# bransonf/mosaic

Hardware: AMD Instinct MI355X
Metric: PIP-join points/sec (whole node) at H3 res 9, 1/2/4/8 MI355X vs CPU host (higher is better)
Workload: dtype f64

## Files before the change

mosaic_amd/csrc/join_binned.h:

```cpp
#pragma once
#include <hip/hip_runtime.h>
#include <stddef.h>
#include <stdint.h>

#include <vector>

#include "join_common.h"
#include "tile_images.h"

namespace binned {

struct Pt {
    double x, y;
};
struct PtRow {
    double x, y;
    long long row;
};
__host__ __device__ inline void set_row(Pt&, int64_t) {}
__host__ __device__ inline void set_row(PtRow& p, int64_t r) { p.row = (long long)r; }
__host__ __device__ inline int64_t row_of(const Pt&, int64_t i) { return i; }
__host__ __device__ inline int64_t row_of(const PtRow& p, int64_t) { return (int64_t)p.row; }
inline const long long* row_map(const Pt*) { return nullptr; }
inline const long long* row_map(const PtRow* p) { return &p->row; }
// ... 47 lines not shown

#define MOSAIC_FP_MIX(h, v) ((h) * 0x100000001b3ULL ^ (uint64_t)(v))
static constexpr uint64_t mosaic_layout_fingerprint() {
    uint64_t h = 0xcbf29ce484222325ULL;
    h = MOSAIC_FP_MIX(h, sizeof(JoinArgs));
    h = MOSAIC_FP_MIX(h, sizeof(StreamArgs));
    h = MOSAIC_FP_MIX(h, sizeof(BngStreamArgs));
    h = MOSAIC_FP_MIX(h, sizeof(binned::Scratch));
    h = MOSAIC_FP_MIX(h, offsetof(binned::Scratch, exact_args));
    h = MOSAIC_FP_MIX(h, offsetof(binned::Scratch, sorted_rows));
    h = MOSAIC_FP_MIX(h, offsetof(binned::Scratch, spin_cap));
    h = MOSAIC_FP_MIX(h, offsetof(binned::Scratch, lookback_failed));
    h = MOSAIC_FP_MIX(h, sizeof(binned::Images));
    h = MOSAIC_FP_MIX(h, offsetof(JoinArgs, res));
    h = MOSAIC_FP_MIX(h, offsetof(JoinArgs, counts));
    return h;
}
#undef MOSAIC_FP_MIX
```

mosaic_amd/csrc/join_common.h:

```cpp
#pragma once
#include <hip/hip_runtime.h>
#include <stdint.h>

#include "bng_device.h"
#include "pip_device.h"
#include "raster.h"
#include "tiles.h"

using namespace mosaic;

static const int64_t kEmptyKey = INT64_MIN;

struct HashEntry {
    int64_t key;
    uint32_t first;
    uint32_t count;
};

__host__ __device__ inline uint64_t mix64(uint64_t h) {
    h ^= h >> 33;
    h *= 0xff51afd7ed558ccdULL;
    h ^= h >> 33;
    h *= 0xc4ceb9fe1a85ec53ULL;
    h ^= h >> 33;
// ... 99 lines not shown
        atomicAdd(&a.counts[key], 1ULL);
    if (PAIRS) {
        unsigned long long idx = atomicAdd(a.pair_count, 1ULL);
        if ((long long)idx < a.pair_cap) {
            a.pair_row[idx] = row;
            a.pair_key[idx] = (int)key;
        }
    }
}

__device__ inline void stage_push(uint32_t* wq, uint32_t& wn, bool mixed, uint32_t rowoff, unsigned long long lt_mask) {
    const unsigned long long mm = __ballot(mixed);
    if (mixed) wq[wn + __popcll(mm & lt_mask)] = rowoff;
    wn += (uint32_t)__popcll(mm);
}
__device__ inline void stage_flush(const JoinArgs& a, uint32_t* wq, uint32_t& wn, int lane, uint32_t min_rows) {
    if (wn < min_rows || wn == 0) return;
    __builtin_amdgcn_fence(__ATOMIC_RELEASE, "wavefront");
    __builtin_amdgcn_wave_barrier();
    __builtin_amdgcn_fence(__ATOMIC_ACQUIRE, "wavefront");
    unsigned long long base = 0;
    if (lane == 0) base = atomicAdd(a.mixq_count, (unsigned long long)wn);
    base = __shfl(base, 0, 64);
    for (uint32_t k = (uint32_t)lane; k < wn; k += 64) a.mixq[base + k] = wq[k];
    __builtin_amdgcn_wave_barrier();
    wn = 0;
}

struct StreamArgs {
    double x0, y0, sxC, syC;
    double gxmax, gymax;
    int32_t cs, qsh, tsh, qs;
    int32_t qnx, tnx;
    int32_t n_quad_words, n_tiles;
    int32_t tb_lds;
    int32_t stage_words;
    const uint32_t* quad;
    const uint32_t* tile_base;
    const uint16_t* csub;
    const uint16_t* blocks;
    uint32_t csub_bytes, blocks_bytes, tile_base_bytes;
    const uint32_t* qrec;
    int32_t n_qrec, n_qrec_words, qrl;
    double sxF, syF, gx0F, gy0F;
    int32_t gxmaxF, gymaxF, fix_ok;
    const uint32_t* tile_lbase;
    const tiles::LineRec* llines;
};
static const int kStageWords = 128;
static const int kCptBufWords = 192;
static const uint32_t kNoLoad = 0x7ffffff0u;

typedef double v2d __attribute__((ext_vector_type(2)));
typedef unsigned int v4u __attribute__((ext_vector_type(4)));

__device__ inline void lds_fill(uint32_t* dst, const uint32_t* __restrict__ src, int n) {
    const int nt = (int)blockDim.x;
    int k = (int)threadIdx.x;
    for (; k + 7 * nt < n; k += 8 * nt) {
        uint32_t v[8];
#pragma unroll
        for (int j = 0; j < 8; j++) v[j] = src[k + j * nt];
#pragma unroll
        for (int j = 0; j < 8; j++) dst[k + j * nt] = v[j];
// ... 14 lines not shown
    return r;
}

template <int SH0 = 0>
__device__ inline uint32_t quad_lookup(const StreamArgs& s, const uint16_t* quad, const uint32_t* qmask,
                                       const uint16_t* qcode, uint32_t ixC, uint32_t iyC) {
    const uint32_t q = quad[mad_u24(iyC >> (s.qsh + SH0), (uint32_t)s.qnx, ixC >> (s.qsh + SH0))];
    const uint32_t r = q - 0x8000u;
    const bool rec = r < (uint32_t)s.n_qrec;
    const uint32_t sh = (uint32_t)(s.cs + s.qrl + SH0);
    const uint32_t b = (__builtin_amdgcn_ubfe(iyC, sh, 3u) << 3) | __builtin_amdgcn_ubfe(ixC, sh, 3u);
    const uint32_t rr = rec ? r : 0u;
    const uint32_t w = qmask[2u * rr + (b >> 5)];
    const uint32_t c = qcode[rr];
    return (rec && __builtin_amdgcn_ubfe(w, b & 31u, 1u)) ? c : q;
}

static const uint32_t kBngPure = 0x80000000u, kBngLeaf = 0x40000000u;
static const uint32_t kBngLdsGather = 0xFFu;
struct BngStreamArgs {
    int32_t e0, n0, ne, nn, C;
    double inv_div, div, f;
    int32_t idiv;
    float ff;
    const uint32_t* cells;
    const uint16_t* leaf;
    uint32_t cells_bytes, leaf_bytes;
    const uint32_t* lcell;
    int32_t lcell_words, lsh, lnx;
    const uint16_t* lvl;
// ... 8 lines not shown
```

mosaic_amd/csrc/join_stream.hip:

```cpp
#include "join_binned.h"
#include "join_common.h"

template <bool LDS_COUNTS, bool PAIRS, bool VEC>
__global__ void __launch_bounds__(1024) __attribute__((amdgpu_waves_per_eu(4))) k_join_stream(JoinArgs a, StreamArgs s) {
    extern __shared__ unsigned int lds[];
    const int nwaves = (int)(blockDim.x >> 6);
    const int ncw = LDS_COUNTS ? a.n_polygons + 64 : 0;
    uint32_t* stage = lds + ncw;
    uint32_t* tb = stage + nwaves * s.stage_words;
    uint32_t* quadw = tb + (s.tb_lds ? s.n_tiles : 0);
    const uint16_t* quad = (const uint16_t*)quadw;
    uint32_t* qmask = quadw + s.n_quad_words;
    const uint16_t* qcode = (const uint16_t*)(qmask + 2 * s.n_qrec);
    lds_fill(quadw, s.quad, s.n_quad_words);
    lds_fill(qmask, s.qrec, s.n_qrec_words);
    if (s.tb_lds)
        lds_fill(tb, s.tile_base, s.n_tiles);
    for (int k = threadIdx.x; k < ncw; k += blockDim.x) lds[k] = 0;
    __syncthreads();
    const __amdgpu_buffer_rsrc_t rsub = stream_rsrc(s.csub, s.csub_bytes);
    const __amdgpu_buffer_rsrc_t rblk = stream_rsrc(s.blocks, s.blocks_bytes);
    const __amdgpu_buffer_rsrc_t rtb = stream_rsrc(s.tile_base, s.tile_base_bytes);
    const int lane = (int)(threadIdx.x & 63);
    const unsigned long long lt_mask = (1ULL << lane) - 1ULL;
    const int wave = __builtin_amdgcn_readfirstlane((int)(threadIdx.x >> 6));
    uint32_t* wq = stage + wave * s.stage_words;
    uint32_t wn = 0;
    const uint32_t cm = (1u << s.cs) - 1u, qm = (1u << s.qs) - 1u, tm = (1u << s.tsh) - 1u;
    const int64_t stride = (int64_t)gridDim.x * blockDim.x * 4;
    int64_t w0 = a.row_lo + ((int64_t)blockIdx.x * blockDim.x + (int64_t)wave * 64) * 4;
    auto row_of = [&](int64_t wb, int k) -> int64_t { return wb + (k >> 1) * 128 + 2 * lane + (k & 1); };
    v2d px[2], py[2];
    auto load4 = [&](int64_t wb) {
        const int64_t r = (wb + 256 <= a.n) ? wb + 2 * lane : a.row_lo;
        px[0] = __builtin_nontemporal_load((const v2d*)(a.x + r));
        px[1] = __builtin_nontemporal_load((const v2d*)(a.x + r + 128));
        py[0] = __builtin_nontemporal_load((const v2d*)(a.y + r));
        py[1] = __builtin_nontemporal_load((const v2d*)(a.y + r + 128));
    };
    if (VEC) load4(w0);
    for (; w0 < a.n; w0 += stride) {
        const bool full = VEC && w0 + 256 <= a.n;
// ... 68 lines not shown
#pragma unroll
        for (int k = 0; k < 4; k++) {
            if (LDS_COUNTS && !PAIRS) {
                const uint32_t slot = code[k] - 1u < 0xfffeu ? code[k] - 1u : (uint32_t)(a.n_polygons + lane);
                atomicAdd(&lds[slot], 1u);
            } else if (code[k] - 1u < 0xfffeu) {
                emit_hit<LDS_COUNTS, PAIRS>(a, row_of(w0, k), code[k] - 1u, lds);
            }
        }
        const bool anym = code[0] == tiles::kMixed || code[1] == tiles::kMixed || code[2] == tiles::kMixed ||
                          code[3] == tiles::kMixed;
        if (__ballot(anym)) {
#pragma unroll
            for (int k = 0; k < 4; k++) {
                const bool m = code[k] == tiles::kMixed;
                const unsigned long long mm = __ballot(m);
                if (m) wq[wn + __popcll(mm & lt_mask)] = (uint32_t)(row_of(w0, k) - a.row_lo);
                wn += (uint32_t)__popcll(mm);
                stage_flush(a, wq, wn, lane, 64);
            }
        }
    }
    stage_flush(a, wq, wn, lane, 1);
    if (LDS_COUNTS) {
        __syncthreads();
        for (int k = threadIdx.x; k < a.n_polygons; k += blockDim.x)
            if (lds[k]) atomicAdd(&a.counts[k], (unsigned long long)lds[k]);
    }
}


template <int aux>
__device__ inline uint32_t gather_b16(__amdgpu_buffer_rsrc_t r, bool need, uint32_t off) {
    uint32_t v = 0u;
    if (need) v = __builtin_amdgcn_raw_buffer_load_b16(r, off, 0, aux);
    return v;
}
__device__ inline uint32_t gather_b32(__amdgpu_buffer_rsrc_t r, bool need, uint32_t off) {
// ... 12 lines not shown
    uint32_t gx[4], gy[4];
    uint32_t tbv[4];
    uint32_t qv[4];
    uint32_t code[4];
    uint32_t leaf[4];
    v4u lrec[4];
};
static const uint32_t kPipeNonFinite = 0x7fffu;
static_assert(tiles::kMaxRasterKeys + 1 < 0x7fff, "key codes stay below kPipeNonFinite");
static const uint32_t kPipeLine = 0x10000u;

template <bool LDS_COUNTS, bool PAIRS>
__global__ void __launch_bounds__(1024) __attribute__((amdgpu_waves_per_eu(4))) k_join_stream_pipe(JoinArgs a, StreamArgs s) {
    extern __shared__ unsigned int lds[];
    const int nwaves = (int)(blockDim.x >> 6);
    const int ncw = LDS_COUNTS ? a.n_polygons + 64 : 0;
    uint32_t* stage = lds + ncw;
    uint32_t* tb = stage + nwaves * s.stage_words;
    uint32_t* quadw = tb + s.n_tiles;
    const uint16_t* quad = (const uint16_t*)quadw;
    uint32_t* qmask = quadw + s.n_quad_words;
    const uint16_t* qcode = (const uint16_t*)(qmask + 2 * s.n_qrec);
    lds_fill(quadw, s.quad, s.n_quad_words);
    lds_fill(qmask, s.qrec, s.n_qrec_words);
    lds_fill(tb, s.tile_base, s.n_tiles);
    for (int k = threadIdx.x; k < ncw; k += blockDim.x) lds[k] = 0;
    __syncthreads();
    const __amdgpu_buffer_rsrc_t rsub = stream_rsrc(s.csub, s.csub_bytes);
    const __amdgpu_buffer_rsrc_t rblk = stream_rsrc(s.blocks, s.blocks_bytes);
    const int lane = (int)(threadIdx.x & 63);
    const unsigned long long lt_mask = (1ULL << lane) - 1ULL;
    const int wave = __builtin_amdgcn_readfirstlane((int)(threadIdx.x >> 6));
    uint32_t* wq = stage + wave * s.stage_words;
    uint32_t wn = 0;
    const uint32_t cm = (1u << s.cs) - 1u, qm = (1u << s.qs) - 1u;
    const double gx0 = -s.x0 * s.sxC, gy0 = -s.y0 * s.syC;
    const uint32_t spill = (uint32_t)(a.n_polygons + lane);
    const int64_t stride = (int64_t)gridDim.x * blockDim.x * 4;
    const int64_t wbase = a.row_lo + ((int64_t)blockIdx.x * blockDim.x + (int64_t)wave * 64) * 4;
    const int64_t T = wbase + 256 <= a.n ? (a.n - 256 - wbase) / stride + 1 : 0;
    auto row_of = [&](int64_t wb, int k) -> int64_t { return wb + (k >> 1) * 128 + 2 * lane + (k & 1); };
    auto stage_a = [&](const double* x, const double* y, const bool* live, bool valid, PipeGroup& g) {
#pragma unroll
        for (int k = 0; k < 4; k++) {
            const bool lv = valid && live[k];
            const uint32_t ixC = min(tiles::fix_cvt(fma(x[k], s.sxF, s.gx0F)), (uint32_t)s.gxmaxF);
            const uint32_t iyC = min(tiles::fix_cvt(fma(y[k], s.syF, s.gy0F)), (uint32_t)s.gymaxF);
            g.gx[k] = ixC;
            g.gy[k] = iyC;
// ... 39 lines not shown
        }
#pragma unroll
        for (int k = 0; k < 4; k++) {
            if (LDS_COUNTS && !PAIRS) {
                const uint32_t slot = min(code[k] - 1u, spill);
                atomicAdd(&lds[slot], 1u);
            } else if (code[k] - 1u < kPipeNonFinite - 1u) {
                emit_hit<LDS_COUNTS, PAIRS>(a, row_of(wb, k), code[k] - 1u, lds);
            }
        }
        const uint32_t cmax = max(max(code[0], code[1]), max(code[2], code[3]));
        if (__ballot(cmax >= kPipeNonFinite)) {
#pragma unroll
            for (int k = 0; k < 4; k++) {
                const bool m = code[k] >= kPipeNonFinite;
                const unsigned long long mm = __ballot(m);
                if (m) wq[wn + __popcll(mm & lt_mask)] = (uint32_t)(row_of(wb, k) - a.row_lo);
                wn += (uint32_t)__popcll(mm);
                stage_flush(a, wq, wn, lane, 64);
            }
        }
    };
    struct Coords {
        v2d px[2], py[2];
    };
    auto load4 = [&](Coords& cb, int64_t wb, bool valid) {
        const int64_t r = valid ? wb + 2 * lane : wbase + 2 * lane;
        cb.px[0] = __builtin_nontemporal_load((const v2d*)(a.x + r));
        cb.px[1] = __builtin_nontemporal_load((const v2d*)(a.x + r + 128));
        cb.py[0] = __builtin_nontemporal_load((const v2d*)(a.y + r));
        cb.py[1] = __builtin_nontemporal_load((const v2d*)(a.y + r + 128));
    };
    Coords cb0, cb1;
    PipeGroup g0, g1;
// ... 35 lines not shown
    if (wt < a.n) {
        double x[4], y[4];
        bool live[4];
#pragma unroll
        for (int k = 0; k < 4; k++) {
            const int64_t r = row_of(wt, k);
            live[k] = r < a.n;
            x[k] = live[k] ? a.x[r] : 0.0;
            y[k] = live[k] ? a.y[r] : 0.0;
        }
        PipeGroup g;
        stage_a(x, y, live, true, g);
        stage_b(g);
        stage_d(g, wt);
    }
    stage_flush(a, wq, wn, lane, 1);
    if (LDS_COUNTS) {
        __syncthreads();
        for (int k = threadIdx.x; k < a.n_polygons; k += blockDim.x)
            if (lds[k]) atomicAdd(&a.counts[k], (unsigned long long)lds[k]);
    }
}


struct CptSet {
    uint32_t a;
    uint32_t b;
    uint32_t c;
    uint32_t code;
    uint32_t leaf;
    v4u lrec;
};

template <bool LDS_COUNTS, bool PAIRS>
__global__ void __launch_bounds__(1024) __attribute__((amdgpu_waves_per_eu(4))) k_join_stream_cpt(JoinArgs a, StreamArgs s) {
    extern __shared__ unsigned int lds[];
    const int nwaves = (int)(blockDim.x >> 6);
    const int ncw = LDS_COUNTS ? a.n_polygons + 64 : 0;
    uint32_t* stage = lds + ncw;
    uint32_t* cbuf_all = stage + nwaves * s.stage_words;
    uint32_t* tb = cbuf_all + nwaves * kCptBufWords;
    uint32_t* quadw = tb + (s.tb_lds ? s.n_tiles : 0);
    const uint16_t* quad = (const uint16_t*)quadw;
    uint32_t* qmask = quadw + s.n_quad_words;
    const uint16_t* qcode = (const uint16_t*)(qmask + 2 * s.n_qrec);
    lds_fill(quadw, s.quad, s.n_quad_words);
    lds_fill(qmask, s.qrec, s.n_qrec_words);
    if (s.tb_lds) lds_fill(tb, s.tile_base, s.n_tiles);
    for (int k = threadIdx.x; k < ncw; k += blockDim.x) lds[k] = 0;
    __syncthreads();
    const __amdgpu_buffer_rsrc_t rsub = stream_rsrc(s.csub, s.csub_bytes);
    const __amdgpu_buffer_rsrc_t rblk = stream_rsrc(s.blocks, s.blocks_bytes);
    const __amdgpu_buffer_rsrc_t rtb = stream_rsrc(s.tile_base, s.tile_base_bytes);
// ... 60 lines not shown
        if (MOSAIC_ABL_GATHER_HIT & 9) z.lrec = v4u{0u, 0u, __float_as_uint(2.0f), 0x00010001u};
        if (MOSAIC_ABL_GATHER_HIT & 10) z.leaf = z.code == kPipeLine ? z.leaf : 1u;
#endif
        const float u = (float)__builtin_amdgcn_ubfe(z.a, 0u, fb) * (1.0f / (float)(1 << F));
        const float v = (float)__builtin_amdgcn_ubfe(z.b, 0u, fb) * (1.0f / (float)(1 << F));
        const float sv = fmaf(__uint_as_float(z.lrec.x), u, fmaf(__uint_as_float(z.lrec.y), v, __uint_as_float(z.lrec.z)));
        const uint32_t pos = z.lrec.w & 0xffffu, neg = z.lrec.w >> 16;
        uint32_t lc = sv >= 1.0f ? pos : (uint32_t)tiles::kMixed;
        lc = sv <= -1.0f ? neg : lc;
        const uint32_t code = z.code == kPipeLine ? lc : (z.code | z.leaf);
        const uint32_t src = (z.a >> 24) & 63u, k = z.a >> 30;
        const int64_t row = wb + (int64_t)((k >> 1) * 128u + 2u * src + (k & 1u));
        answer(code, row);
        const bool m = code >= kPipeNonFinite;
        if (__ballot(m)) {
            const unsigned long long mm = __ballot(m);
            if (m) wq[wn + __popcll(mm & lt_mask)] = (uint32_t)(row - a.row_lo);
            wn += (uint32_t)__popcll(mm);
            stage_flush(a, wq, wn, lane, 64);
        }
    };
    auto stage_a = [&](const double* x, const double* y, const bool* live, bool valid, CptSet& z, CptSet& z2, bool& two,
                       int64_t wb) {
        uint32_t fa[4], fb[4], fc[4];
        bool pend[4];
#pragma unroll
        for (int k = 0; k < 4; k++) {
            const uint32_t ixC = min(tiles::fix_cvt(fma(x[k], s.sxF, gx0v)), (uint32_t)s.gxmaxF);
            const uint32_t iyC = min(tiles::fix_cvt(fma(y[k], s.syF, gy0v)), (uint32_t)s.gymaxF);
            const uint32_t q0 = quad_lookup<F>(s, quad, qmask, qcode, ixC, iyC);
            const uint32_t q = valid && live[k] ? q0 : 0u;
            const uint32_t tile = mad_u24(iyC >> (s.tsh + F), (uint32_t)s.tnx, ixC >> (s.tsh + F));
            if (LDS_COUNTS && !PAIRS) atomicAdd(&lds[min(q - 1u, spill)], 1u);
            else if (q - 1u < kPipeNonFinite - 1u) emit_hit<LDS_COUNTS, PAIRS>(a, wb + (k >> 1) * 128 + 2 * lane + (k & 1), q - 1u, lds);
// ... 102 lines not shown
            const int64_t r = wt + (k >> 1) * 128 + 2 * lane + (k & 1);
            live[k] = r < a.n;
            x[k] = live[k] ? a.x[r] : 0.0;
            y[k] = live[k] ? a.y[r] : 0.0;
        }
        CptSet z, z2;
        bool two = false;
        stage_a(x, y, live, true, z, z2, two, wt);
        set_b(z);
        set_d(z, wt);
        if (two) {
            set_b(z2);
            set_d(z2, wt);
        }
    }
    stage_flush(a, wq, wn, lane, 1);
    if (LDS_COUNTS) {
        __syncthreads();
        for (int k = threadIdx.x; k < a.n_polygons; k += blockDim.x)
            if (lds[k]) atomicAdd(&a.counts[k], (unsigned long long)lds[k]);
    }
}

template <bool LDS_COUNTS, bool PAIRS, bool VEC>
__global__ void __launch_bounds__(1024) __attribute__((amdgpu_waves_per_eu(4))) k_join_stream_bng(JoinArgs a, BngStreamArgs s) {
    extern __shared__ unsigned int lds[];
    const int ncw = LDS_COUNTS ? a.n_polygons + 64 : 0;
    uint32_t* stage = lds + ncw;
    uint32_t* lcw = stage + (int)(blockDim.x >> 6) * kStageWords;
    const uint8_t* lcell = (const uint8_t*)lcw;
    const bool use_lc = s.lcell_words > 0;
// ... 368 lines not shown
        for (int k = threadIdx.x; k < a.n_polygons; k += blockDim.x)
            if (lds[k]) atomicAdd(&a.counts[k], (unsigned long long)lds[k]);
    }
}

template <bool LDS_COUNTS, bool PAIRS>
__global__ void __launch_bounds__(256) k_join_leaf(JoinArgs a, StreamArgs s, uint32_t* q2, unsigned long long* q2_count) {
    extern __shared__ unsigned int lds[];
    if (LDS_COUNTS) {
        for (int k = threadIdx.x; k < a.n_polygons; k += blockDim.x) lds[k] = 0;
        __syncthreads();
    }
    JoinArgs aq = a;
    aq.mixq = q2;
    aq.mixq_count = q2_count;
    uint32_t* wq = lds + (LDS_COUNTS ? a.n_polygons : 0) + (threadIdx.x >> 6) * kStageWords;
    uint32_t wn = 0;
    constexpr int F = tiles::kFixBits;
    const int lane = (int)(threadIdx.x & 63);
    const unsigned long long lt_mask = (1ULL << lane) - 1ULL;
    const uint16_t* quad = (const uint16_t*)s.quad;
    const uint32_t* qmask = s.qrec;
    const uint16_t* qcode = (const uint16_t*)(s.qrec + 2 * s.n_qrec);
    const uint32_t cs = (uint32_t)s.cs, qs = (uint32_t)s.qs, cm = (1u << cs) - 1u, qm = (1u << qs) - 1u;
    const unsigned long long total = *a.mixq_count;
    const unsigned long long stride = (unsigned long long)gridDim.x * blockDim.x;
    for (unsigned long long t0 = (unsigned long long)blockIdx.x * blockDim.x + (threadIdx.x & ~63u); t0 < total; t0 += stride) {
        const unsigned long long t = t0 + (unsigned long long)lane;
        const bool live = t < total;
        const uint32_t off = live ? a.mixq[t] : 0u;
        const int64_t row = a.row_lo + (int64_t)off;
        uint32_t code = tiles::kMixed;
        if (live) {
            const double x = a.x[row], y = a.y[row];
            if (isfinite(x + y)) {
                const uint32_t gix = min(tiles::fix_cvt(fma(x, s.sxF, s.gx0F)), (uint32_t)s.gxmaxF);
                const uint32_t giy = min(tiles::fix_cvt(fma(y, s.syF, s.gy0F)), (uint32_t)s.gymaxF);
                const uint32_t ixC = gix >> F, iyC = giy >> F, ix = ixC >> cs, iy = iyC >> cs;
                const uint32_t q = quad_lookup<F>(s, quad, qmask, qcode, gix, giy);
                const uint32_t e = q < 0x8000u ? q : s.csub[((q & 0x7fffu) << (2 * qs)) + (((iy & qm) << qs) | (ix & qm))];
                code = e;
                if (tiles::sub_is_block(e) && !(e & tiles::kLineBit)) {
                    const uint32_t tile = (iyC >> s.tsh) * (uint32_t)s.tnx + (ixC >> s.tsh);
                    const uint32_t base = s.tile_base[tile];
                    const uint32_t lc = s.blocks[base + ((e & 0x3fffu) << (2 * cs)) + (((iyC & cm) << cs) | (ixC & cm))];
                    code = lc;
                    if (tiles::leaf_is_line(lc)) {
                        const tiles::LineRec lr = s.llines[s.tile_lbase[tile] + (lc & 0x3fffu)];
                        const uint32_t fm = (1u << (cs + F)) - 1u;
                        const float sc = 1.0f / (float)(1 << F);
                        code = tiles::line_code(lr, (float)(gix & fm) * sc, (float)(giy & fm) * sc);
                    }
                } else if (tiles::sub_is_block(e)) {
                    code = tiles::kMixed;
                }
            }
        }
        const bool keep = live && code >= 0x8000u;
        if (live && !keep && code != 0u) {
            if (LDS_COUNTS && !PAIRS) atomicAdd(&lds[code - 1u], 1u);
            else emit_hit<LDS_COUNTS, PAIRS>(a, row, code - 1u, lds);
        }
        stage_push(wq, wn, keep, off, lt_mask);
        stage_flush(aq, wq, wn, lane, 64);
    }
    stage_flush(aq, wq, wn, lane, 1);
    if (LDS_COUNTS) {
        __syncthreads();
        for (int k = threadIdx.x; k < a.n_polygons; k += blockDim.x)
            if (lds[k]) atomicAdd(&a.counts[k], (unsigned long long)lds[k]);
    }
}

const void* leaf_kernel(bool lds, bool pairs) {
    if (pairs) return (const void*)k_join_leaf<false, true>;
    if (lds) return (const void*)k_join_leaf<true, false>;
    return (const void*)k_join_leaf<false, false>;
}

// ... 29 lines not shown
```

mosaic_amd/csrc/mosaic_hip.hip:

```cpp
#include <hip/hip_runtime.h>
#include <hipcub/hipcub.hpp>
#include <stdint.h>
#include <stdio.h>
#include <string.h>

#include <sys/syscall.h>
#include <unistd.h>

#include <algorithm>
#include <atomic>
#include <chrono>
#include <memory>
#include <mutex>
#include <numeric>
#include <string>
#include <sys/mman.h>
#include <dirent.h>
#include <sys/prctl.h>
#include <thread>
#include <unordered_map>
#include <vector>

#include "../../include/mosaic_hip.h"
#include "bng_device.h"
// ... 1785 lines not shown
    int block = 256;
    int blocks_per_cu = 8;
    int raster = 16;
    int raster_adaptive = 1;
    int raster_min_segments = 0;
    int lane_edges = 0;
    int tiles = 1;
    int point_raster = 1;
    int raster_sub = 64;
    int raster_cell = 16;
    int raster_quad = 1;
    int raster_lines = 1;
    int raster_tb_lds = 1;
    int raster_leaf_lines = 1;
    int leaf_join = 1;
    int leaf_blocks_per_cu = 2;
    int exact_defer = 0;
    int raster_build = 1;
    int raster_quad_records = 1;
    int stream_block = 1024;
    int bng_cpt = 1;
    int stream_pipe = 2;
    int bng_lds = 1;
    int bng_cell = 32;
    int bng_group_lines = 1;
    int bng_wedges = 1;
    int cell_blocks_per_cu = 256;
    int mixed_blocks_per_cu = 16;
    int mixed_rows = 1;
    int64_t host_chunk = (int64_t)1 << 25;
    int timing = 0;
// ... 538 lines not shown
        o.raster_quad = (int)v;
    } else if (k == "raster_adaptive") {
        o.raster_adaptive = v ? 1 : 0;
    } else if (k == "raster_min_segments") {
        if (v < 0 || v > 1000000) return fail(MOSAIC_E_ARG, "raster_min_segments must be in [0, 1e6]");
        o.raster_min_segments = (int)v;
    } else if (k == "raster_lines") {
        o.raster_lines = v ? 1 : 0;
    } else if (k == "raster_tb_lds") {
        if (v < 0 || v > 2) return fail(MOSAIC_E_ARG, "raster_tb_lds must be 0, 1 or 2");
        o.raster_tb_lds = (int)v;
    } else if (k == "raster_leaf_lines") {
        o.raster_leaf_lines = v ? 1 : 0;
    } else if (k == "leaf_join") {
        o.leaf_join = v ? 1 : 0;
    } else if (k == "exact_defer") {
        o.exact_defer = v ? 1 : 0;
    } else if (k == "leaf_blocks_per_cu") {
        if (v < 1 || v > 64) return fail(MOSAIC_E_ARG, "leaf_blocks_per_cu must be in [1, 64]");
        o.leaf_blocks_per_cu = (int)v;
    } else if (k == "raster_quad_records") {
        o.raster_quad_records = v ? 1 : 0;
    } else if (k == "raster_build") {
        if (v < 0 || v > 2) return fail(MOSAIC_E_ARG, "raster_build must be 0 (host), 1 (GPU) or 2 (GPU, lane-per-sub-block lines)");
        o.raster_build = (int)v;
    } else if (k == "host_chunk") {
        if (v < 0) return fail(MOSAIC_E_ARG, "host_chunk must be >= 0");
        o.host_chunk = v;
    } else if (k == "stream_block") {
        if (v < 64 || v > 1024 || v % 64) return fail(MOSAIC_E_ARG, "stream_block must be a multiple of 64 in [64, 1024]");
// ... 1644 lines not shown
    a.rowmap = nullptr;
    bool lds = ch->n_polygons <= kLdsCountsMax;
    size_t shm = lds ? (size_t)ch->n_polygons * 4 : 0;
    int g = grid_size(c, n);
    bool binned_used = false, exact_inline = false;
    if (n > 0) {
        hipEvent_t tstop;
        if ((rc = timing_begin(c, &tstop))) return rc;
        const bool h3g = ch->grid == MOSAIC_GRID_H3;
#define MOSAIC_LAUNCH(KERNEL, SHM) hipLaunchKernelGGL(KERNEL, dim3(g), dim3(c->block), SHM, c->stream, a)
        const bool tiled = h3g && c->tiles && ch->tiles_ok;
        const bool praster = tiled && c->point_raster && ch->raster_ok;
        const bool bngdense = !h3g && c->tiles && ch->bng_ok;
        StreamArgs sa = ch->stream;
        const int blk = c->stream_block;
        size_t shm_s = (lds && !pairs ? ((size_t)ch->n_polygons + 64) * 4 : 0) + (size_t)(blk / 64) * sa.stage_words * 4 +
                       (size_t)sa.n_quad_words * 4 + (size_t)sa.n_qrec_words * 4;
        sa.tb_lds = ch->tb_lds_budget && shm_s + (size_t)sa.n_tiles * 4 <= kStreamLdsMax ? 1 : 0;
        if (sa.tb_lds) shm_s += (size_t)sa.n_tiles * 4;
        const bool stream = praster && ch->stream_ok && shm_s <= kStreamLdsMax;
        binned_used = tiled && !stream && c->bin_points && n >= c->bin_min_rows;
        if (bngdense) {
            a.bng_cells = (const uint32_t*)ch->bng_cells.p;
            a.bng_e0 = ch->bng_e0;
            a.bng_n0 = ch->bng_n0;
            a.bng_ne = ch->bng_ne;
            a.bng_nn = ch->bng_nn;
            a.bng_div = ch->bng_div;
            a.bng_leaf = (const uint16_t*)ch->bng_leaf.p;
            a.bng_C = ch->bng_C;
            a.bng_wedge = ch->bng_C > 0 && ch->bng_wedges ? 1 : 0;
// ... 59 lines not shown
        else hipLaunchKernelGGL((k_join_mixed_bng<false, false, R_>), dim3(gm), dim3(c->block), 0, c->stream, ac); \
    } while (0)
                hipEvent_t mstop = nullptr;
                if (c->timing == 2 && lo == 0 && (rc = timing_begin(c, &mstop))) return rc;
                if (c->mixed_rows == 4) MOSAIC_MIXED_BNG(4);
                else if (c->mixed_rows == 2) MOSAIC_MIXED_BNG(2);
                else MOSAIC_MIXED_BNG(1);
#undef MOSAIC_MIXED_BNG
                if (mstop) HIP_TRY(hipEventRecord(mstop, c->stream));
                HIP_TRY(hipGetLastError());
            }
            tstop = nullptr;
        } else if (stream) {
            const int64_t chunk = ((int64_t)1 << 32) - 256;
            const int64_t rows = std::min<int64_t>(n, chunk);
            if ((rc = c->mix_queue.reserve((size_t)rows * 4 + 16))) return rc;
            a.mixq = (uint32_t*)c->mix_queue.p;
            a.mixq_count = sc + 4;
            const bool leafq = c->leaf_join && sa.llines && sa.fix_ok;
            if (leafq && (rc = c->mix_queue2.reserve((size_t)rows * 4 + 16))) return rc;
            a.exact_inline = c->exact_defer ? 0 : 1;
            exact_inline = !c->exact_defer;
            const bool aligned = (((uintptr_t)dx | (uintptr_t)dy) & 15) == 0;
            auto mode_for = [&](bool vec) -> int {
                int mode = vec && sa.fix_ok ? c->stream_pipe : 0;
                if (mode >= 2 && !(sa.cs + tiles::kFixBits + sa.qs <= 24 && sa.tsh + tiles::kFixBits <= 24 && sa.n_tiles <= 65536 &&
                                   shm_s + (size_t)(blk / 64) * kCptBufWords * 4 <= kStreamLdsMax))
                    mode = 1;
                if (mode == 1 && !sa.tb_lds) mode = 0;
                return mode;
            };
            auto kernel_for = [&](bool vec) -> const void* { return stream_kernel_h3(mode_for(vec), lds, pairs, vec); };
            auto shm_for = [&](bool vec) -> size_t {
                return shm_s + (mode_for(vec) >= 2 ? (size_t)(blk / 64) * kCptBufWords * 4 : 0);
            };
            int per_cu = 0;
            if (hipOccupancyMaxActiveBlocksPerMultiprocessor(&per_cu, kernel_for(true), blk, shm_for(true)) != hipSuccess ||
                per_cu < 1)
                per_cu = 1;
            for (int64_t lo = 0; lo < n; lo += chunk) {
                JoinArgs ac = a;
                ac.row_lo = lo;
                ac.n = std::min<int64_t>(n, lo + chunk);
                const void* kfn = kernel_for(aligned && ac.n - lo >= 256);
                const int mode = mode_for(aligned && ac.n - lo >= 256);
                if (lo == 0) {
                    static const char* const names[3] = {"k_join_stream", "k_join_stream_pipe", "k_join_stream_cpt"};
                    c->last_kernel = names[mode];
                }
                if (lo > 0) HIP_TRY(hipMemsetAsync(ac.mixq_count, 0, 8, c->stream));
// ... 3 lines not shown
                HIP_TRY(hipLaunchKernel(kfn, dim3(gs), dim3(blk), kargs, shm_for(aligned && ac.n - lo >= 256), c->stream));
                if (tstop && lo == 0) HIP_TRY(hipEventRecord(tstop, c->stream));
                const int gm = (int)std::max<int64_t>(1, std::min<int64_t>((ac.n - lo + 4 * c->block - 1) / (4 * c->block),
                                                                           (int64_t)c->n_cu * c->mixed_blocks_per_cu));
#define MOSAIC_MIXED(KERNEL, SHM) \
    hipLaunchKernelGGL(KERNEL, dim3(gm), dim3(c->block), SHM, c->stream, ac)
                hipEvent_t mstop = nullptr;
                if (c->timing == 2 && lo == 0 && (rc = timing_begin(c, &mstop))) return rc;
                const int lb = leafq ? std::max(1, c->n_cu * c->leaf_blocks_per_cu) : 0;
                if (leafq) {
                    uint32_t* q2 = (uint32_t*)c->mix_queue2.p;
                    unsigned long long* q2c = sc + 7;
                    if (lo > 0) HIP_TRY(hipMemsetAsync(q2c, 0, 8, c->stream));
                    void* largs[] = {&ac, &sa, &q2, &q2c};
                    HIP_TRY(hipLaunchKernel(leaf_kernel(lds, pairs), dim3((unsigned)lb), dim3(256), largs,
                                            (lds && !pairs ? shm : 0) + 4 * kStageWords * 4, c->stream));
                    ac.mixq = q2;
                    ac.mixq_count = q2c;
                }
                if (c->mixed_rows == 4) {
                    if (pairs) MOSAIC_MIXED((k_join_mixed<false, true, 4>), 0);
                    else if (lds) MOSAIC_MIXED((k_join_mixed<true, false, 4>), shm);
                    else MOSAIC_MIXED((k_join_mixed<false, false, 4>), 0);
                } else if (c->mixed_rows == 2) {
                    if (pairs) MOSAIC_MIXED((k_join_mixed<false, true, 2>), 0);
                    else if (lds) MOSAIC_MIXED((k_join_mixed<true, false, 2>), shm);
                    else MOSAIC_MIXED((k_join_mixed<false, false, 2>), 0);
                } else {
                    if (pairs) MOSAIC_MIXED((k_join_mixed<false, true, 1>), 0);
                    else if (lds) MOSAIC_MIXED((k_join_mixed<true, false, 1>), shm);
                    else MOSAIC_MIXED((k_join_mixed<false, false, 1>), 0);
// ... 1520 lines not shown
```

mosaic_amd/csrc/tiles.h:

```cpp
#pragma once
#include <math.h>
#include <stdint.h>

#include "h3_device.h"
#include "raster.h"
#include "raster_build.h"

#include <algorithm>
#include <atomic>
#include <functional>
#include <thread>
#include <vector>

namespace mosaic {
namespace tiles {

static const uint32_t kSkip = 0;
static const uint32_t kFull = 1;

static const uint16_t kMixed = 0xffffu;
static const uint16_t kSubBlock = 0x8000u;
static const uint16_t kLineBit = 0x4000u;
static const int32_t kMaxRasterKeys = 0x7ffd;

// ... 103 lines not shown
    const uint32_t n = e & 0x3fffu;
    if (e & kLineBit) {
        const uint32_t fm = (1u << (r.sshift + r.cshift + F)) - 1u;
        const float sc = 1.0f / (float)(1 << F);
        return line_code(*(const LineRec*)(r.blocks + base - 8 * (size_t)(n + 1)), (float)((uint32_t)gix & fm) * sc,
                         (float)((uint32_t)giy & fm) * sc);
    }
    const uint16_t lc = r.blocks[base + ((size_t)n << (2 * r.cshift)) + (size_t)(((iyC & cm) << r.cshift) | (ixC & cm))];
    if (leaf_is_line(lc) && r.llines) {
        const uint32_t fm = (1u << (r.cshift + F)) - 1u;
        const float sc = 1.0f / (float)(1 << F);
        return line_code(r.llines[r.tile_lbase[(iy >> r.sshift) * r.tnx + (ix >> r.sshift)] + (lc & 0x3fffu)],
                         (float)((uint32_t)gix & fm) * sc, (float)((uint32_t)giy & fm) * sc);
    }
    return leaf_is_line(lc) ? kMixed : lc;
}

template <class T>
struct NoInitAlloc : std::allocator<T> {
    template <class U>
    struct rebind {
        using other = NoInitAlloc<U>;
    };
    NoInitAlloc() = default;
    template <class U>
    NoInitAlloc(const NoInitAlloc<U>&) noexcept {}
    template <class U>
    void construct(U* p) noexcept {
        ::new ((void*)p) U;
    }
// ... 399 lines not shown
```

Baseline: 314.6 billion.

## Tag mixed-row queue entries with tile and leaf to skip leaf re-lookup

Stream kernels now push a (row offset, tag) pair into the mixed queue, where the tag encodes the tile index and the line leaf code already found during streaming. The leaf-join kernel uses the tag to go straight to the line record, skipping the quad/csub/block lookups. Rows tagged as fully mixed are passed through without touching their coordinates. This doubles queue bytes and stage LDS, enlarges the leaf-kernel staging buffer, and lowers leaf blocks per CU from 2 to 1.

```diff
diff --git a/mosaic_amd/csrc/join_binned.h b/mosaic_amd/csrc/join_binned.h
--- a/mosaic_amd/csrc/join_binned.h
+++ b/mosaic_amd/csrc/join_binned.h
@@ -85,6 +85,8 @@
     h = MOSAIC_FP_MIX(h, sizeof(binned::Images));
     h = MOSAIC_FP_MIX(h, offsetof(JoinArgs, res));
     h = MOSAIC_FP_MIX(h, offsetof(JoinArgs, counts));
+    h = MOSAIC_FP_MIX(h, offsetof(StreamArgs, tagq));
+    h = MOSAIC_FP_MIX(h, offsetof(StreamArgs, tile_lbase));
     return h;
 }
 #undef MOSAIC_FP_MIX
diff --git a/mosaic_amd/csrc/join_common.h b/mosaic_amd/csrc/join_common.h
--- a/mosaic_amd/csrc/join_common.h
+++ b/mosaic_amd/csrc/join_common.h
@@ -137,18 +137,26 @@
     if (mixed) wq[wn + __popcll(mm & lt_mask)] = rowoff;
     wn += (uint32_t)__popcll(mm);
 }
-__device__ inline void stage_flush(const JoinArgs& a, uint32_t* wq, uint32_t& wn, int lane, uint32_t min_rows) {
+__device__ inline void stage_push2(uint32_t* wq, uint32_t& wn, bool mixed, uint32_t rowoff, uint32_t tag,
+                                   unsigned long long lt_mask) {
+    const unsigned long long mm = __ballot(mixed);
+    if (mixed) *(uint2*)(wq + 2u * (wn + (uint32_t)__popcll(mm & lt_mask))) = make_uint2(rowoff, tag);
+    wn += (uint32_t)__popcll(mm);
+}
+__device__ inline void stage_flush(const JoinArgs& a, uint32_t* wq, uint32_t& wn, int lane, uint32_t min_rows, uint32_t ew = 1u) {
     if (wn < min_rows || wn == 0) return;
     __builtin_amdgcn_fence(__ATOMIC_RELEASE, "wavefront");
     __builtin_amdgcn_wave_barrier();
     __builtin_amdgcn_fence(__ATOMIC_ACQUIRE, "wavefront");
     unsigned long long base = 0;
     if (lane == 0) base = atomicAdd(a.mixq_count, (unsigned long long)wn);
-    base = __shfl(base, 0, 64);
-    for (uint32_t k = (uint32_t)lane; k < wn; k += 64) a.mixq[base + k] = wq[k];
+    base = __shfl(base, 0, 64) * ew;
+    for (uint32_t k = (uint32_t)lane; k < wn * ew; k += 64) a.mixq[base + k] = wq[k];
     __builtin_amdgcn_wave_barrier();
     wn = 0;
 }
+
+__host__ __device__ inline int stream_count_words(int n_polygons) { return (n_polygons + 64 + 1) & ~1; }
 
 struct StreamArgs {
     double x0, y0, sxC, syC;
@@ -167,10 +175,16 @@
     int32_t n_qrec, n_qrec_words, qrl;
     double sxF, syF, gx0F, gy0F;
     int32_t gxmaxF, gymaxF, fix_ok;
+    int32_t tagq;
     const uint32_t* tile_lbase;
     const tiles::LineRec* llines;
 };
 static const int kStageWords = 128;
+__device__ inline uint32_t stage_flush_rows(int32_t stage_words, uint32_t ew) {
+    const int32_t r = stage_words / (int32_t)ew - 64;
+    return (uint32_t)(r < 1 ? 1 : r);
+}
+static const int kLeafStageWords = 320;
 static const int kCptBufWords = 192;
 static const uint32_t kNoLoad = 0x7ffffff0u;
 
@@ -215,6 +229,39 @@
     const uint32_t w = qmask[2u * rr + (b >> 5)];
     const uint32_t c = qcode[rr];
     return (rec && __builtin_amdgcn_ubfe(w, b & 31u, 1u)) ? c : q;
+}
+
+__device__ inline uint32_t leaf_row_code(const StreamArgs& s, uint32_t tag, double x, double y) {
+    constexpr int F = tiles::kFixBits;
+    const uint32_t t = tiles::tagged_code_fixed(s.tile_lbase, s.llines, s.cs, s.sxF, s.gx0F, s.syF, s.gy0F, (uint32_t)s.gxmaxF,
+                                                (uint32_t)s.gymaxF, tag, x, y);
+    if (t != (uint32_t)tiles::kSubBlock) return t;
+    if (!isfinite(x + y)) return tiles::kMixed;
+    const uint16_t* quad = (const uint16_t*)s.quad;
+    const uint32_t* qmask = s.qrec;
+    const uint16_t* qcode = (const uint16_t*)(s.qrec + 2 * s.n_qrec);
+    const uint32_t cs = (uint32_t)s.cs, qs = (uint32_t)s.qs, cm = (1u << cs) - 1u, qm = (1u << qs) - 1u;
+    const uint32_t gix = min(tiles::fix_cvt(fma(x, s.sxF, s.gx0F)), (uint32_t)s.gxmaxF);
+    const uint32_t giy = min(tiles::fix_cvt(fma(y, s.syF, s.gy0F)), (uint32_t)s.gymaxF);
+    const uint32_t ixC = gix >> F, iyC = giy >> F, ix = ixC >> cs, iy = iyC >> cs;
+    const uint32_t q = quad_lookup<F>(s, quad, qmask, qcode, gix, giy);
+    const uint32_t e = q < 0x8000u ? q : s.csub[((q & 0x7fffu) << (2 * qs)) + (((iy & qm) << qs) | (ix & qm))];
+    uint32_t code = e;
+    if (tiles::sub_is_block(e) && !(e & tiles::kLineBit)) {
+        const uint32_t tile = (iyC >> s.tsh) * (uint32_t)s.tnx + (ixC >> s.tsh);
+        const uint32_t base = s.tile_base[tile];
+        const uint32_t lc = s.blocks[base + ((e & 0x3fffu) << (2 * cs)) + (((iyC & cm) << cs) | (ixC & cm))];
+        code = lc;
+        if (tiles::leaf_is_line(lc)) {
+            const tiles::LineRec lr = s.llines[s.tile_lbase[tile] + (lc & 0x3fffu)];
+            const uint32_t fm = (1u << (cs + F)) - 1u;
+            const float sc = 1.0f / (float)(1 << F);
+            code = tiles::line_code(lr, (float)(gix & fm) * sc, (float)(giy & fm) * sc);
+        }
+    } else if (tiles::sub_is_block(e)) {
+        code = tiles::kMixed;
+    }
+    return code;
 }
 
 static const uint32_t kBngPure = 0x80000000u, kBngLeaf = 0x40000000u;
diff --git a/mosaic_amd/csrc/join_stream.hip b/mosaic_amd/csrc/join_stream.hip
--- a/mosaic_amd/csrc/join_stream.hip
+++ b/mosaic_amd/csrc/join_stream.hip
@@ -5,7 +5,7 @@
 __global__ void __launch_bounds__(1024) __attribute__((amdgpu_waves_per_eu(4))) k_join_stream(JoinArgs a, StreamArgs s) {
     extern __shared__ unsigned int lds[];
     const int nwaves = (int)(blockDim.x >> 6);
-    const int ncw = LDS_COUNTS ? a.n_polygons + 64 : 0;
+    const int ncw = LDS_COUNTS ? stream_count_words(a.n_polygons) : 0;
     uint32_t* stage = lds + ncw;
     uint32_t* tb = stage + nwaves * s.stage_words;
     uint32_t* quadw = tb + (s.tb_lds ? s.n_tiles : 0);
@@ -26,6 +26,7 @@
     const int wave = __builtin_amdgcn_readfirstlane((int)(threadIdx.x >> 6));
     uint32_t* wq = stage + wave * s.stage_words;
     uint32_t wn = 0;
+    const uint32_t ew = s.tagq ? 2u : 1u, fl = stage_flush_rows(s.stage_words, ew);
     const uint32_t cm = (1u << s.cs) - 1u, qm = (1u << s.qs) - 1u, tm = (1u << s.tsh) - 1u;
     const int64_t stride = (int64_t)gridDim.x * blockDim.x * 4;
     int64_t w0 = a.row_lo + ((int64_t)blockIdx.x * blockDim.x + (int64_t)wave * 64) * 4;
@@ -124,14 +125,14 @@
 #pragma unroll
             for (int k = 0; k < 4; k++) {
                 const bool m = code[k] == tiles::kMixed;
-                const unsigned long long mm = __ballot(m);
-                if (m) wq[wn + __popcll(mm & lt_mask)] = (uint32_t)(row_of(w0, k) - a.row_lo);
-                wn += (uint32_t)__popcll(mm);
-                stage_flush(a, wq, wn, lane, 64);
-            }
-        }
-    }
-    stage_flush(a, wq, wn, lane, 1);
+                const uint32_t off = (uint32_t)(row_of(w0, k) - a.row_lo);
+                if (s.tagq) stage_push2(wq, wn, m, off, tiles::kTagUnknown, lt_mask);
+                else stage_push(wq, wn, m, off, lt_mask);
+                stage_flush(a, wq, wn, lane, fl, ew);
+            }
+        }
+    }
+    stage_flush(a, wq, wn, lane, 1, ew);
     if (LDS_COUNTS) {
         __syncthreads();
         for (int k = threadIdx.x; k < a.n_polygons; k += blockDim.x)
@@ -174,7 +175,7 @@
 __global__ void __launch_bounds__(1024) __attribute__((amdgpu_waves_per_eu(4))) k_join_stream_pipe(JoinArgs a, StreamArgs s) {
     extern __shared__ unsigned int lds[];
     const int nwaves = (int)(blockDim.x >> 6);
-    const int ncw = LDS_COUNTS ? a.n_polygons + 64 : 0;
+    const int ncw = LDS_COUNTS ? stream_count_words(a.n_polygons) : 0;
     uint32_t* stage = lds + ncw;
     uint32_t* tb = stage + nwaves * s.stage_words;
     uint32_t* quadw = tb + s.n_tiles;
@@ -193,6 +194,7 @@
     const int wave = __builtin_amdgcn_readfirstlane((int)(threadIdx.x >> 6));
     uint32_t* wq = stage + wave * s.stage_words;
     uint32_t wn = 0;
+    const uint32_t ew = s.tagq ? 2u : 1u, fl = stage_flush_rows(s.stage_words, ew);
     const uint32_t cm = (1u << s.cs) - 1u, qm = (1u << s.qs) - 1u;
     const double gx0 = -s.x0 * s.sxC, gy0 = -s.y0 * s.syC;
     const uint32_t spill = (uint32_t)(a.n_polygons + lane);
@@ -262,10 +264,15 @@
 #pragma unroll
             for (int k = 0; k < 4; k++) {
                 const bool m = code[k] >= kPipeNonFinite;
-                const unsigned long long mm = __ballot(m);
-                if (m) wq[wn + __popcll(mm & lt_mask)] = (uint32_t)(row_of(wb, k) - a.row_lo);
-                wn += (uint32_t)__popcll(mm);
-                stage_flush(a, wq, wn, lane, 64);
+                const uint32_t off = (uint32_t)(row_of(wb, k) - a.row_lo);
+                if (s.tagq) {
+                    const uint32_t sh = (uint32_t)(s.tsh + tiles::kFixBits);
+                    const uint32_t tile = __umul24(g.gy[k] >> sh, (uint32_t)s.tnx) + (g.gx[k] >> sh);
+                    stage_push2(wq, wn, m, off, tiles::queue_tag(tile, g.code[k] == 0u ? g.leaf[k] : (uint32_t)tiles::kMixed), lt_mask);
+                } else {
+                    stage_push(wq, wn, m, off, lt_mask);
+                }
+                stage_flush(a, wq, wn, lane, fl, ew);
             }
         }
     };
@@ -331,7 +338,7 @@
         stage_b(g);
         stage_d(g, wt);
     }
-    stage_flush(a, wq, wn, lane, 1);
+    stage_flush(a, wq, wn, lane, 1, ew);
     if (LDS_COUNTS) {
         __syncthreads();
         for (int k = threadIdx.x; k < a.n_polygons; k += blockDim.x)
@@ -353,7 +360,7 @@
 __global__ void __launch_bounds__(1024) __attribute__((amdgpu_waves_per_eu(4))) k_join_stream_cpt(JoinArgs a, StreamArgs s) {
     extern __shared__ unsigned int lds[];
     const int nwaves = (int)(blockDim.x >> 6);
-    const int ncw = LDS_COUNTS ? a.n_polygons + 64 : 0;
+    const int ncw = LDS_COUNTS ? stream_count_words(a.n_polygons) : 0;
     uint32_t* stage = lds + ncw;
     uint32_t* cbuf_all = stage + nwaves * s.stage_words;
     uint32_t* tb = cbuf_all + nwaves * kCptBufWords;
@@ -444,10 +451,13 @@
         answer(code, row);
         const bool m = code >= kPipeNonFinite;
         if (__ballot(m)) {
-            const unsigned long long mm = __ballot(m);
-            if (m) wq[wn + __popcll(mm & lt_mask)] = (uint32_t)(row - a.row_lo);
-            wn += (uint32_t)__popcll(mm);
-            stage_flush(a, wq, wn, lane, 64);
+            if (s.tagq)
+                stage_push2(wq, wn, m, (uint32_t)(row - a.row_lo),
+                            tiles::queue_tag(z.c >> 16, z.code == 0u ? z.leaf : (uint32_t)tiles::kMixed), lt_mask);
+            else
+                stage_push(wq, wn, m, (uint32_t)(row - a.row_lo), lt_mask);
+            const uint32_t ew = s.tagq ? 2u : 1u;
+            stage_flush(a, wq, wn, lane, stage_flush_rows(s.stage_words, ew), ew);
         }
     };
     auto stage_a = [&](const double* x, const double* y, const bool* live, bool valid, CptSet& z, CptSet& z2, bool& two,
@@ -580,7 +590,7 @@
             set_d(z2, wt);
         }
     }
-    stage_flush(a, wq, wn, lane, 1);
+    stage_flush(a, wq, wn, lane, 1, s.tagq ? 2u : 1u);
     if (LDS_COUNTS) {
         __syncthreads();
         for (int k = threadIdx.x; k < a.n_polygons; k += blockDim.x)
@@ -979,55 +989,32 @@
     JoinArgs aq = a;
     aq.mixq = q2;
     aq.mixq_count = q2_count;
-    uint32_t* wq = lds + (LDS_COUNTS ? a.n_polygons : 0) + (threadIdx.x >> 6) * kStageWords;
+    uint32_t* wq = lds + (LDS_COUNTS ? a.n_polygons : 0) + (threadIdx.x >> 6) * kLeafStageWords;
     uint32_t wn = 0;
-    constexpr int F = tiles::kFixBits;
     const int lane = (int)(threadIdx.x & 63);
     const unsigned long long lt_mask = (1ULL << lane) - 1ULL;
-    const uint16_t* quad = (const uint16_t*)s.quad;
-    const uint32_t* qmask = s.qrec;
-    const uint16_t* qcode = (const uint16_t*)(s.qrec + 2 * s.n_qrec);
-    const uint32_t cs = (uint32_t)s.cs, qs = (uint32_t)s.qs, cm = (1u << cs) - 1u, qm = (1u << qs) - 1u;
     const unsigned long long total = *a.mixq_count;
     const unsigned long long stride = (unsigned long long)gridDim.x * blockDim.x;
     for (unsigned long long t0 = (unsigned long long)blockIdx.x * blockDim.x + (threadIdx.x & ~63u); t0 < total; t0 += stride) {
         const unsigned long long t = t0 + (unsigned long long)lane;
         const bool live = t < total;
-        const uint32_t off = live ? a.mixq[t] : 0u;
+        uint32_t off = 0u, tag = tiles::kTagUnknown;
+        if (live && s.tagq) {
+            const uint2 e = ((const uint2*)a.mixq)[t];
+            off = e.x, tag = e.y;
+        } else if (live) {
+            off = a.mixq[t];
+        }
         const int64_t row = a.row_lo + (int64_t)off;
         uint32_t code = tiles::kMixed;
-        if (live) {
-            const double x = a.x[row], y = a.y[row];
-            if (isfinite(x + y)) {
-                const uint32_t gix = min(tiles::fix_cvt(fma(x, s.sxF, s.gx0F)), (uint32_t)s.gxmaxF);
-                const uint32_t giy = min(tiles::fix_cvt(fma(y, s.syF, s.gy0F)), (uint32_t)s.gymaxF);
-                const uint32_t ixC = gix >> F, iyC = giy >> F, ix = ixC >> cs, iy = iyC >> cs;
-                const uint32_t q = quad_lookup<F>(s, quad, qmask, qcode, gix, giy);
-                const uint32_t e = q < 0x8000u ? q : s.csub[((q & 0x7fffu) << (2 * qs)) + (((iy & qm) << qs) | (ix & qm))];
-                code = e;
-                if (tiles::sub_is_block(e) && !(e & tiles::kLineBit)) {
-                    const uint32_t tile = (iyC >> s.tsh) * (uint32_t)s.tnx + (ixC >> s.tsh);
-                    const uint32_t base = s.tile_base[tile];
-                    const uint32_t lc = s.blocks[base + ((e & 0x3fffu) << (2 * cs)) + (((iyC & cm) << cs) | (ixC & cm))];
-                    code = lc;
-                    if (tiles::leaf_is_line(lc)) {
-                        const tiles::LineRec lr = s.llines[s.tile_lbase[tile] + (lc & 0x3fffu)];
-                        const uint32_t fm = (1u << (cs + F)) - 1u;
-                        const float sc = 1.0f / (float)(1 << F);
-                        code = tiles::line_code(lr, (float)(gix & fm) * sc, (float)(giy & fm) * sc);
-                    }
-                } else if (tiles::sub_is_block(e)) {
-                    code = tiles::kMixed;
-                }
-            }
-        }
+        if (live && (tag & 0xffffu) != (uint32_t)tiles::kMixed) code = leaf_row_code(s, tag, a.x[row], a.y[row]);
         const bool keep = live && code >= 0x8000u;
         if (live && !keep && code != 0u) {
             if (LDS_COUNTS && !PAIRS) atomicAdd(&lds[code - 1u], 1u);
             else emit_hit<LDS_COUNTS, PAIRS>(a, row, code - 1u, lds);
         }
         stage_push(wq, wn, keep, off, lt_mask);
-        stage_flush(aq, wq, wn, lane, 64);
+        stage_flush(aq, wq, wn, lane, kLeafStageWords - 64);
     }
     stage_flush(aq, wq, wn, lane, 1);
     if (LDS_COUNTS) {
diff --git a/mosaic_amd/csrc/mosaic_hip.hip b/mosaic_amd/csrc/mosaic_hip.hip
--- a/mosaic_amd/csrc/mosaic_hip.hip
+++ b/mosaic_amd/csrc/mosaic_hip.hip
@@ -1823,7 +1823,8 @@
     int raster_tb_lds = 1;
     int raster_leaf_lines = 1;
     int leaf_join = 1;
-    int leaf_blocks_per_cu = 2;
+    int leaf_blocks_per_cu = 1;
+    int queue_tags = 1;
     int exact_defer = 0;
     int raster_build = 1;
     int raster_quad_records = 1;
@@ -2392,6 +2393,8 @@
         o.raster_leaf_lines = v ? 1 : 0;
     } else if (k == "leaf_join") {
         o.leaf_join = v ? 1 : 0;
+    } else if (k == "queue_tags") {
+        o.queue_tags = v ? 1 : 0;
     } else if (k == "exact_defer") {
         o.exact_defer = v ? 1 : 0;
     } else if (k == "leaf_blocks_per_cu") {
@@ -4066,7 +4069,7 @@
         const bool bngdense = !h3g && c->tiles && ch->bng_ok;
         StreamArgs sa = ch->stream;
         const int blk = c->stream_block;
-        size_t shm_s = (lds && !pairs ? ((size_t)ch->n_polygons + 64) * 4 : 0) + (size_t)(blk / 64) * sa.stage_words * 4 +
+        size_t shm_s = (lds && !pairs ? (size_t)stream_count_words(ch->n_polygons) * 4 : 0) + (size_t)(blk / 64) * sa.stage_words * 4 +
                        (size_t)sa.n_quad_words * 4 + (size_t)sa.n_qrec_words * 4;
         sa.tb_lds = ch->tb_lds_budget && shm_s + (size_t)sa.n_tiles * 4 <= kStreamLdsMax ? 1 : 0;
         if (sa.tb_lds) shm_s += (size_t)sa.n_tiles * 4;
@@ -4156,10 +4159,11 @@
         } else if (stream) {
             const int64_t chunk = ((int64_t)1 << 32) - 256;
             const int64_t rows = std::min<int64_t>(n, chunk);
-            if ((rc = c->mix_queue.reserve((size_t)rows * 4 + 16))) return rc;
+            const bool leafq = c->leaf_join && sa.llines && sa.fix_ok;
+            sa.tagq = leafq && c->queue_tags ? 1 : 0;
+            if ((rc = c->mix_queue.reserve((size_t)rows * (sa.tagq ? 8 : 4) + 16))) return rc;
             a.mixq = (uint32_t*)c->mix_queue.p;
             a.mixq_count = sc + 4;
-            const bool leafq = c->leaf_join && sa.llines && sa.fix_ok;
             if (leafq && (rc = c->mix_queue2.reserve((size_t)rows * 4 + 16))) return rc;
             a.exact_inline = c->exact_defer ? 0 : 1;
             exact_inline = !c->exact_defer;
@@ -4176,6 +4180,10 @@
             auto shm_for = [&](bool vec) -> size_t {
                 return shm_s + (mode_for(vec) >= 2 ? (size_t)(blk / 64) * kCptBufWords * 4 : 0);
             };
+            if (sa.tagq && std::max(shm_for(true), shm_for(false)) + (size_t)(blk / 64) * kStageWords * 4 <= kStreamLdsMax) {
+                shm_s += (size_t)(blk / 64) * kStageWords * 4;
+                sa.stage_words = 2 * kStageWords;
+            }
             int per_cu = 0;
             if (hipOccupancyMaxActiveBlocksPerMultiprocessor(&per_cu, kernel_for(true), blk, shm_for(true)) != hipSuccess ||
                 per_cu < 1)
@@ -4209,7 +4217,7 @@
                     if (lo > 0) HIP_TRY(hipMemsetAsync(q2c, 0, 8, c->stream));
                     void* largs[] = {&ac, &sa, &q2, &q2c};
                     HIP_TRY(hipLaunchKernel(leaf_kernel(lds, pairs), dim3((unsigned)lb), dim3(256), largs,
-                                            (lds && !pairs ? shm : 0) + 4 * kStageWords * 4, c->stream));
+                                            (lds && !pairs ? shm : 0) + 4 * kLeafStageWords * 4, c->stream));
                     ac.mixq = q2;
                     ac.mixq_count = q2c;
                 }
diff --git a/mosaic_amd/csrc/tiles.h b/mosaic_amd/csrc/tiles.h
--- a/mosaic_amd/csrc/tiles.h
+++ b/mosaic_amd/csrc/tiles.h
@@ -141,6 +141,25 @@
                          (float)((uint32_t)gix & fm) * sc, (float)((uint32_t)giy & fm) * sc);
     }
     return leaf_is_line(lc) ? kMixed : lc;
+}
+
+static const uint32_t kTagUnknown = 0u;
+MOSAIC_HD uint32_t queue_tag(uint32_t tile, uint32_t leaf) {
+    if (!leaf_is_line(leaf)) return kMixed;
+    return tile <= 0xffffu ? (tile << 16) | leaf : kTagUnknown;
+}
+MOSAIC_HD uint16_t tagged_code_fixed(const uint32_t* tile_lbase, const LineRec* llines, int cshift, double ax, double bx,
+                                     double ay, double by, uint32_t gxmax, uint32_t gymax, uint32_t tag, double x, double y) {
+    const uint32_t lc = tag & 0xffffu;
+    if (lc == kMixed) return kMixed;
+    if (!leaf_is_line(lc)) return kSubBlock;
+    const uint32_t lbase = tile_lbase[tag >> 16];
+    uint32_t gix = fix_cvt(fma(x, ax, bx)), giy = fix_cvt(fma(y, ay, by));
+    gix = gix > gxmax ? gxmax : gix;
+    giy = giy > gymax ? gymax : giy;
+    const uint32_t fm = (1u << (cshift + kFixBits)) - 1u;
+    const float sc = 1.0f / (float)(1 << kFixBits);
+    return line_code(llines[lbase + (lc & 0x3fffu)], (float)(gix & fm) * sc, (float)(giy & fm) * sc);
 }
 
 template <class T>
```

Measured after the change: 316.1 billion (median of 2 runs). No clear change (+0.5%).
